# HengyiWang/spann3r

Hardware: NVIDIA H100
Metric: frames/sec (512x384, 10-frame seq) enc->mem-attn->dec->DPT (higher is better)
Workload: dtype bf16x3 (split-bf16 operands, fp32 accumulate; tf32 attention)

## Files before the change

### spann3r_b200/csrc/attention.cu

```cuda
#include "common.cuh"
#include "kernels.cuh"
#include "wgmma.cuh"

#include <cstdlib>
#include <cstring>

namespace s3r {

namespace attn {
constexpr int BQ = 128;
constexpr int BKV = 128;
constexpr int D = 64;
constexpr int Q_BYTES = BQ * D * 4;
constexpr int K_BYTES = BKV * D * 4;
constexpr int V_BYTES = D * BKV * 4;
constexpr int KV_STAGES = 3;
constexpr int SMEM = Q_BYTES + KV_STAGES * (K_BYTES + V_BYTES) + 1024 + 256;
constexpr int kThreads = 384;
constexpr int kConsumerWarps = 8;
}

__global__ void __launch_bounds__(attn::kThreads, 1) attention_kernel(const __grid_constant__ AttnArgs args) {
  using namespace attn;
  extern __shared__ uint8_t smem_raw[];
  uint8_t* smem = smem_raw + ((1024u - (smem_u32(smem_raw) & 1023u)) & 1023u);
  uint8_t* sQ = smem;
  uint8_t* sKV = sQ + Q_BYTES;
  uint64_t* bars = reinterpret_cast<uint64_t*>(sKV + KV_STAGES * (K_BYTES + V_BYTES));
  uint64_t* q_full = bars;
  uint64_t* kv_full = bars + 1;
  uint64_t* kv_empty = bars + 1 + KV_STAGES;

  const int warp = threadIdx.x >> 5, lane = threadIdx.x & 31;
  const int q0 = blockIdx.x * BQ;
  const int bh = blockIdx.y;
  const int nblk = (args.nk + BKV - 1) / BKV;

  if (warp == 0 && lane == 0) {
    tma_prefetch_desc(&args.tmQ);
    tma_prefetch_desc(&args.tmK);
    tma_prefetch_desc(&args.tmV);
    mbar_init(q_full, 1);
    for (int i = 0; i < KV_STAGES; ++i) {
      mbar_init(&kv_full[i], 1);
      mbar_init(&kv_empty[i], kConsumerWarps);
    }
    fence_barrier_init();
  }
  __syncthreads();
  pdl_launch_dependents();
  pdl_wait();

  if (warp < 4) {
    asm volatile("setmaxnreg.dec.sync.aligned.u32 40;");
    if (warp == 0 && lane == 0) {
      mbar_arrive_expect_tx(q_full, Q_BYTES);
      tma_load_3d(sQ, &args.tmQ, q_full, 0, q0, bh);
      tma_load_3d(sQ + Q_BYTES / 2, &args.tmQ, q_full, 32, q0, bh);
      for (int j = 0; j < nblk; ++j) {
        const int st = j % KV_STAGES;
        const uint32_t ph = (j / KV_STAGES) & 1;
        mbar_wait(&kv_empty[st], ph ^ 1);
        uint8_t* k = sKV + st * (K_BYTES + V_BYTES);
        uint8_t* v = k + K_BYTES;
        mbar_arrive_expect_tx(&kv_full[st], K_BYTES + V_BYTES);
        tma_load_3d(k, &args.tmK, &kv_full[st], 0, j * BKV, bh);
        tma_load_3d(k + K_BYTES / 2, &args.tmK, &kv_full[st], 32, j * BKV, bh);
#pragma unroll
        for (int a = 0; a < 4; ++a) tma_load_3d(v + a * (V_BYTES / 4), &args.tmV, &kv_full[st], j * BKV + a * 32, 0, bh);
      }
    }
    return;
  }

  asm volatile("setmaxnreg.inc.sync.aligned.u32 232;");
  const int wg = (warp - 4) >> 2;
  const int wq = warp & 3;
  const int g = lane >> 2, t4 = lane & 3;
  const uint32_t aQ = __shfl_sync(0xffffffffu, smem_u32(sQ), 0) + wg * (64 * 128);
  const uint32_t aKV = __shfl_sync(0xffffffffu, smem_u32(sKV), 0);
  constexpr float kLog2e = 1.4426950408889634f;

  float o[32];
#pragma unroll
  for (int i = 0; i < 32; ++i) o[i] = 0.f;
  float m0 = -INFINITY, m1 = -INFINITY, l0 = 0.f, l1 = 0.f;
  const int src_lo = (lane & ~3) | (t4 >> 1), src_hi = src_lo + 2;
  const bool odd = (t4 & 1) != 0;

  mbar_wait(q_full, 0);
  for (int j = 0; j < nblk; ++j) {
    const int st = j % KV_STAGES;
    mbar_wait(&kv_full[st], (j / KV_STAGES) & 1);
    const uint32_t aK = aKV + st * (K_BYTES + V_BYTES);
    const uint32_t aV = aK + K_BYTES;

    float s[64];
    wgmma_fence();
#pragma unroll
    for (int kk = 0; kk < 8; ++kk) {
      const uint32_t part = (kk >> 2) * (Q_BYTES / 2), ko = (kk & 3) * 2;
      wgmma_tf32_n128_ss(s, wgmma_desc_sw128_kmajor(aQ + part) + ko, wgmma_desc_sw128_kmajor(aK + part) + ko, kk > 0);
    }
    wgmma_commit();
    wgmma_wait<0>();

    const int kbase = j * BKV;
    if (kbase + BKV > args.nk) {
#pragma unroll
      for (int i = 0; i < 16; ++i) {
        const int c = kbase + 8 * i + 2 * t4;
        if (c >= args.nk) { s[4 * i] = -INFINITY; s[4 * i + 2] = -INFINITY; }
        if (c + 1 >= args.nk) { s[4 * i + 1] = -INFINITY; s[4 * i + 3] = -INFINITY; }
      }
    }
    float b0 = -INFINITY, b1 = -INFINITY;
#pragma unroll
    for (int i = 0; i < 16; ++i) {
      b0 = fmaxf(b0, fmaxf(s[4 * i], s[4 * i + 1]));
      b1 = fmaxf(b1, fmaxf(s[4 * i + 2], s[4 * i + 3]));
    }
#pragma unroll
    for (int x = 1; x < 4; x <<= 1) {
      b0 = fmaxf(b0, __shfl_xor_sync(0xffffffffu, b0, x));
      b1 = fmaxf(b1, __shfl_xor_sync(0xffffffffu, b1, x));
    }
    const float n0 = fmaxf(m0, b0), n1 = fmaxf(m1, b1);
    const float al0 = (j == 0) ? 0.f : exp2f((m0 - n0) * kLog2e);
    const float al1 = (j == 0) ? 0.f : exp2f((m1 - n1) * kLog2e);
    m0 = n0;
    m1 = n1;
    const float nr0 = -n0 * kLog2e, nr1 = -n1 * kLog2e;
    float ps0 = 0.f, ps1 = 0.f;
#pragma unroll
    for (int i = 0; i < 64; ++i) {
      const bool r1 = (i & 2) != 0;
      const float e = exp2f(fmaf(s[i], kLog2e, r1 ? nr1 : nr0));
      const uint32_t rb = (__float_as_uint(e) + 0x1000u) & 0xffffe000u;
      s[i] = __uint_as_float(rb);
      if (r1) ps1 += s[i]; else ps0 += s[i];
    }
    l0 = l0 * al0 + ps0;
    l1 = l1 * al1 + ps1;
#pragma unroll
    for (int i = 0; i < 8; ++i) {
      o[4 * i] *= al0; o[4 * i + 1] *= al0;
      o[4 * i + 2] *= al1; o[4 * i + 3] *= al1;
    }

    uint32_t pa[16][4];
#pragma unroll
    for (int kk = 0; kk < 16; ++kk) {
      const float x0 = __shfl_sync(0xffffffffu, s[4 * kk], src_lo), x1 = __shfl_sync(0xffffffffu, s[4 * kk + 1], src_lo);
      const float y0 = __shfl_sync(0xffffffffu, s[4 * kk + 2], src_lo), y1 = __shfl_sync(0xffffffffu, s[4 * kk + 3], src_lo);
      const float z0 = __shfl_sync(0xffffffffu, s[4 * kk], src_hi), z1 = __shfl_sync(0xffffffffu, s[4 * kk + 1], src_hi);
      const float w0 = __shfl_sync(0xffffffffu, s[4 * kk + 2], src_hi), w1 = __shfl_sync(0xffffffffu, s[4 * kk + 3], src_hi);
      pa[kk][0] = __float_as_uint(odd ? x1 : x0);
      pa[kk][1] = __float_as_uint(odd ? y1 : y0);
      pa[kk][2] = __float_as_uint(odd ? z1 : z0);
      pa[kk][3] = __float_as_uint(odd ? w1 : w0);
    }
    wgmma_fence();
#pragma unroll
    for (int kk = 0; kk < 16; ++kk)
      wgmma_tf32_n64_rs(o, pa[kk], wgmma_desc_sw128_kmajor(aV + (kk >> 2) * (V_BYTES / 4)) + (kk & 3) * 2, 1);
    wgmma_commit();
    wgmma_wait<0>();
    __syncwarp();
    if (lane == 0) mbar_arrive(&kv_empty[st]);
  }

#pragma unroll
  for (int x = 1; x < 4; x <<= 1) {
    l0 += __shfl_xor_sync(0xffffffffu, l0, x);
    l1 += __shfl_xor_sync(0xffffffffu, l1, x);
  }
  const float inv0 = 1.0f / l0, inv1 = 1.0f / l1;
  const int b = bh / args.heads, h = bh - b * args.heads;
#pragma unroll
  for (int r = 0; r < 2; ++r) {
    const int q = q0 + wg * 64 + wq * 16 + g + 8 * r;
    if (q >= args.nq) continue;
    const float inv = r ? inv1 : inv0;
    const long long row = ((long long)b * args.nq + q) * args.ldo + h * D;
#pragma unroll
    for (int i = 0; i < 8; ++i) {
      const float x = o[4 * i + 2 * r] * inv, y = o[4 * i + 2 * r + 1] * inv;
      const long long off = row + 8 * i + 2 * t4;
      if (args.o_f32) *reinterpret_cast<float2*>(args.o_f32 + off) = make_float2(x, y);
      if (args.o_hi) {
        uint32_t hh, ll;
        split2_bf16(x, y, hh, ll);
        *reinterpret_cast<uint32_t*>(args.o_hi + off) = hh;
        *reinterpret_cast<uint32_t*>(args.o_lo + off) = ll;
      }
    }
  }
}

int attn_plan_init(AttnPlan* plan, const float* q, const float* k, const float* vt, int BH, int heads, int nq, int nk,
                   int nk_pad) {
  using namespace attn;
  memset(plan, 0, sizeof(*plan));
  if (nk_pad % 4 != 0 || nk_pad < nk) {
    set_error("attention: nk_pad=%d must be >= nk=%d and a multiple of 4", nk_pad, nk);
    return -1;
  }
  AttnArgs& a = plan->args;
  {
    uint64_t dims[3] = {64, (uint64_t)nq, (uint64_t)BH};
    uint64_t str[2] = {64 * 4, (uint64_t)nq * 64 * 4};
    uint32_t box[3] = {32, (uint32_t)BQ, 1};
    int r = encode_tmap(&a.tmQ, CU_TENSOR_MAP_DATA_TYPE_FLOAT32, 3, q, dims, str, box);
    if (r) return r;
  }
  {
    uint64_t dims[3] = {64, (uint64_t)nk, (uint64_t)BH};
    uint64_t str[2] = {64 * 4, (uint64_t)nk * 64 * 4};
    uint32_t box[3] = {32, (uint32_t)BKV, 1};
    int r = encode_tmap(&a.tmK, CU_TENSOR_MAP_DATA_TYPE_FLOAT32, 3, k, dims, str, box);
    if (r) return r;
  }
  {
    uint64_t dims[3] = {(uint64_t)nk, 64, (uint64_t)BH};
    uint64_t str[2] = {(uint64_t)nk_pad * 4, (uint64_t)nk_pad * 64 * 4};
    uint32_t box[3] = {32, 64, 1};
    int r = encode_tmap(&a.tmV, CU_TENSOR_MAP_DATA_TYPE_FLOAT32, 3, vt, dims, str, box);
    if (r) return r;
  }
  a.nq = nq; a.nk = nk; a.heads = heads;
  plan->grid = dim3((nq + BQ - 1) / BQ, BH);
  plan->flops = 4.0 * BH * (double)nq * nk * 64;
  return 0;
}

static int attn_launch_args(const AttnPlan& plan, const AttnArgs& a, cudaStream_t st) {
  using namespace attn;
  static PerDeviceOnce once;
  bool& attr_set = once.cur();
  if (!attr_set) {
    cudaError_t e = cudaFuncSetAttribute(attention_kernel, cudaFuncAttributeMaxDynamicSharedMemorySize, SMEM);
    if (e != cudaSuccess) {
      set_error("attention: cudaFuncSetAttribute(smem=%d): %s", SMEM, cudaGetErrorString(e));
      return -5;
    }
    attr_set = true;
  }
  cudaError_t e = launch_pdl(attention_kernel, plan.grid, dim3(kThreads), SMEM, st, a);
  if (e != cudaSuccess) {
    set_error("attention launch failed: %s", cudaGetErrorString(e));
    return -6;
  }
  return 0;
}

int attn_launch(const AttnPlan& plan, __nv_bfloat16* o_hi, __nv_bfloat16* o_lo, float* o_f32, long long ldo,
                cudaStream_t st) {
  AttnArgs a = plan.args;
  a.o_hi = o_hi; a.o_lo = o_lo; a.o_f32 = o_f32; a.ldo = ldo;
  return attn_launch_args(plan, a, st);
}

int launch_attention(const float* q, const float* k, const float* vt, int BH, int heads, int nq, int nk, int nk_pad,
                     __nv_bfloat16* o_hi, __nv_bfloat16* o_lo, float* o_f32, long long ldo, cudaStream_t st) {
  if (heads <= 0 || BH % heads != 0 || ldo % 2 != 0) {
    set_error("attention: bh=%d must be a multiple of heads=%d, and ldo=%lld even (paired stores)", BH, heads, ldo);
    return -1;
  }
  if (nq <= 0 || nk <= 0 || BH <= 0) return 0;
  AttnPlan plan;
  int r = attn_plan_init(&plan, q, k, vt, BH, heads, nq, nk, nk_pad);
  if (r) return r;
  return attn_launch(plan, o_hi, o_lo, o_f32, ldo, st);
}

}
```

### spann3r_b200/csrc/common.cuh

```cuda
#pragma once
#include <cuda.h>
#include <cuda_bf16.h>
#include <cuda_runtime.h>
#include <stdint.h>

#include <cstdlib>
#include <utility>

namespace s3r {

__device__ __forceinline__ uint32_t smem_u32(const void* p) {
  return static_cast<uint32_t>(__cvta_generic_to_shared(p));
}
__device__ __forceinline__ uint32_t lane_id() { return threadIdx.x & 31; }
__device__ __forceinline__ bool elect_one() {
  uint32_t pred = 0;
  asm volatile(
      "{\n\t.reg .pred P1;\n\t"
      "elect.sync _|P1, 0xffffffff;\n\t"
      "selp.u32 %0, 1, 0, P1;\n\t}\n"
      : "=r"(pred));
  return pred != 0;
}

__device__ __forceinline__ void split_bf16(float x, __nv_bfloat16& hi, __nv_bfloat16& lo) {
  hi = __float2bfloat16_rn(x);
  lo = __float2bfloat16_rn(x - __bfloat162float(hi));
}
__device__ __forceinline__ void split2_bf16(float a, float b, uint32_t& hi, uint32_t& lo) {
  const __nv_bfloat162 h = __floats2bfloat162_rn(a, b);
  const uint32_t hu = *reinterpret_cast<const uint32_t*>(&h);
  const float ah = __uint_as_float(hu << 16), bh = __uint_as_float(hu & 0xffff0000u);
  const __nv_bfloat162 l = __floats2bfloat162_rn(a - ah, b - bh);
  hi = hu;
  lo = *reinterpret_cast<const uint32_t*>(&l);
}
__device__ __forceinline__ uint32_t pack_bf16(__nv_bfloat16 a, __nv_bfloat16 b) {
  return (uint32_t)__bfloat16_as_ushort(a) | ((uint32_t)__bfloat16_as_ushort(b) << 16);
}
__device__ __forceinline__ float to_tf32(float x) {
  uint32_t r;
  asm("cvt.rna.tf32.f32 %0, %1;" : "=r"(r) : "f"(x));
  return __uint_as_float(r);
}
__device__ __forceinline__ float gelu_erf1(float x) {
  return 0.5f * x * (1.0f + erff(x * 0.70710678118654752440f));
}
static __device__ __noinline__ float4 gelu_erf4(float4 x) {
  return make_float4(gelu_erf1(x.x), gelu_erf1(x.y), gelu_erf1(x.z), gelu_erf1(x.w));
}

__device__ __forceinline__ void mbar_init(uint64_t* bar, uint32_t count) {
  asm volatile("mbarrier.init.shared::cta.b64 [%0], %1;" ::"r"(smem_u32(bar)), "r"(count));
}
__device__ __forceinline__ void fence_barrier_init() {
  asm volatile("fence.mbarrier_init.release.cluster;" ::: "memory");
}
__device__ __forceinline__ void mbar_arrive_expect_tx(uint64_t* bar, uint32_t bytes) {
  asm volatile("mbarrier.arrive.expect_tx.shared::cta.b64 _, [%0], %1;" ::"r"(smem_u32(bar)), "r"(bytes)
               : "memory");
}
__device__ __forceinline__ void mbar_arrive(uint64_t* bar) {
  asm volatile("mbarrier.arrive.shared::cta.b64 _, [%0];" ::"r"(smem_u32(bar)) : "memory");
}
__device__ __forceinline__ bool mbar_try_wait(uint64_t* bar, uint32_t parity) {
  uint32_t ok;
  asm volatile(
      "{\n\t.reg .pred P1;\n\t"
      "mbarrier.try_wait.parity.shared::cta.b64 P1, [%1], %2;\n\t"
      "selp.u32 %0, 1, 0, P1;\n\t}\n"
      : "=r"(ok)
      : "r"(smem_u32(bar)), "r"(parity)
      : "memory");
  return ok != 0;
}
__device__ __forceinline__ void mbar_wait(uint64_t* bar, uint32_t parity) {
  uint32_t spins = 0;
  while (!mbar_try_wait(bar, parity)) {
    if (++spins > (1u << 28)) { asm volatile("trap;"); }
  }
}

__device__ __forceinline__ void fence_proxy_async_smem() {
  asm volatile("fence.proxy.async.shared::cta;" ::: "memory");
}
__device__ __forceinline__ void tma_prefetch_desc(const CUtensorMap* m) {
  asm volatile("prefetch.tensormap [%0];" ::"l"(reinterpret_cast<uint64_t>(m)) : "memory");
}
__device__ __forceinline__ void tma_load_2d(void* smem, const CUtensorMap* m, uint64_t* bar, int c0, int c1) {
  asm volatile(
      "cp.async.bulk.tensor.2d.shared::cta.global.mbarrier::complete_tx::bytes [%0], [%1, {%3, %4}], [%2];" ::"r"(
          smem_u32(smem)),
      "l"(reinterpret_cast<uint64_t>(m)), "r"(smem_u32(bar)), "r"(c0), "r"(c1)
      : "memory");
}
__device__ __forceinline__ void tma_load_3d(void* smem, const CUtensorMap* m, uint64_t* bar, int c0, int c1,
                                            int c2) {
  asm volatile(
      "cp.async.bulk.tensor.3d.shared::cta.global.mbarrier::complete_tx::bytes [%0], [%1, {%3, %4, %5}], [%2];" ::
          "r"(smem_u32(smem)),
      "l"(reinterpret_cast<uint64_t>(m)), "r"(smem_u32(bar)), "r"(c0), "r"(c1), "r"(c2)
      : "memory");
}
__device__ __forceinline__ void tma_load_4d(void* smem, const CUtensorMap* m, uint64_t* bar, int c0, int c1,
                                            int c2, int c3) {
  asm volatile(
      "cp.async.bulk.tensor.4d.shared::cta.global.mbarrier::complete_tx::bytes [%0], [%1, {%3, %4, %5, %6}], "
      "[%2];" ::"r"(smem_u32(smem)),
      "l"(reinterpret_cast<uint64_t>(m)), "r"(smem_u32(bar)), "r"(c0), "r"(c1), "r"(c2), "r"(c3)
      : "memory");
}

__device__ __forceinline__ void mbar_arrive_expect_tx_u(uint32_t bar, uint32_t bytes) {
  asm volatile("mbarrier.arrive.expect_tx.shared::cta.b64 _, [%0], %1;" ::"r"(bar), "r"(bytes) : "memory");
}
__device__ __forceinline__ void tma_load_3d_u(uint32_t smem, const CUtensorMap* m, uint32_t bar, int c0, int c1, int c2) {
  asm volatile(
      "cp.async.bulk.tensor.3d.shared::cta.global.mbarrier::complete_tx::bytes [%0], [%1, {%3, %4, %5}], [%2];" ::
          "r"(smem),
      "l"(reinterpret_cast<uint64_t>(m)), "r"(bar), "r"(c0), "r"(c1), "r"(c2)
      : "memory");
}
__device__ __forceinline__ void tma_load_4d_u(uint32_t smem, const CUtensorMap* m, uint32_t bar, int c0, int c1, int c2,
                                              int c3) {
  asm volatile(
      "cp.async.bulk.tensor.4d.shared::cta.global.mbarrier::complete_tx::bytes [%0], [%1, {%3, %4, %5, %6}], "
      "[%2];" ::"r"(smem),
      "l"(reinterpret_cast<uint64_t>(m)), "r"(bar), "r"(c0), "r"(c1), "r"(c2), "r"(c3)
      : "memory");
}

__device__ __forceinline__ uint64_t wgmma_desc_sw128_kmajor(uint32_t smem_addr) {
  uint64_t d = 0;
  d |= (uint64_t)((smem_addr & 0x3FFFF) >> 4);
  d |= (uint64_t)1 << 16;
  d |= (uint64_t)64 << 32;
  d |= (uint64_t)1 << 62;
  return d;
}

__device__ __forceinline__ uint64_t wgmma_desc_sw64_kmajor(uint32_t smem_addr) {
  uint64_t d = 0;
  d |= (uint64_t)((smem_addr & 0x3FFFF) >> 4);
  d |= (uint64_t)1 << 16;
  d |= (uint64_t)32 << 32;
  d |= (uint64_t)2 << 62;
  return d;
}

__device__ __forceinline__ void pdl_launch_dependents() { asm volatile("griddepcontrol.launch_dependents;" ::: "memory"); }
__device__ __forceinline__ void pdl_wait() { asm volatile("griddepcontrol.wait;" ::: "memory"); }

__device__ __forceinline__ unsigned long long globaltimer_ns() {
  unsigned long long t;
  asm volatile("mov.u64 %0, %%globaltimer;" : "=l"(t));
  return t;
}

__device__ __forceinline__ void st_f4(float* p, float a, float b, float c, float d) {
  *reinterpret_cast<float4*>(p) = make_float4(a, b, c, d);
}

struct PerDeviceOnce {
  bool done[64] = {};
  bool& cur() {
    int d = 0;
    cudaGetDevice(&d);
    return done[d & 63];
  }
};

template <typename... KArgs, typename... Args>
inline cudaError_t launch_pdl(void (*kernel)(KArgs...), dim3 grid, dim3 block, size_t smem, cudaStream_t st, Args&&... args) {
  cudaLaunchConfig_t cfg = {};
  cfg.gridDim = grid;
  cfg.blockDim = block;
  cfg.dynamicSmemBytes = smem;
  cfg.stream = st;
  static const bool use_pdl = (getenv("S3R_NO_PDL") == nullptr);
  cudaLaunchAttribute attr[1];
  attr[0].id = cudaLaunchAttributeProgrammaticStreamSerialization;
  attr[0].val.programmaticStreamSerializationAllowed = 1;
  cfg.attrs = attr;
  cfg.numAttrs = use_pdl ? 1 : 0;
  return cudaLaunchKernelEx(&cfg, kernel, std::forward<Args>(args)...);
}

}
```

### spann3r_b200/csrc/kernels.cuh

```cuda
#pragma once
#include <cuda_bf16.h>
#include <cuda_runtime.h>

#include "gemm.cuh"
#include <cuda.h>

struct s3r_loss_desc;
struct s3r_attn_train_desc;

namespace s3r {

int launch_split(const float* x, long long ldx, __nv_bfloat16* hi, __nv_bfloat16* lo, long long ldp, int col0,
                 long long rows, int C, int relu, cudaStream_t st);
int launch_split_stats(const float* x, long long ldx, long long rows, int C, float* out, long long ldo, __nv_bfloat16* hi,
                       __nv_bfloat16* lo, long long ldp, float2* stats, cudaStream_t st);
int launch_layernorm(const float* x, long long ldx, const float* w, const float* b, long long wb_group_stride,
                     long long rows_per_group, float eps, long long rows, int C, float* out, long long ldo,
                     __nv_bfloat16* hi, __nv_bfloat16* lo, long long ldp, int col0, long long swap_rows,
                     cudaStream_t st);
int launch_im2col_patch16(const float* img, long long sb, long long sc, long long sy, long long sx, int B, int gh,
                          int gw, __nv_bfloat16* hi, __nv_bfloat16* lo, cudaStream_t st);
int launch_im2col_3x3s2(const __nv_bfloat16* ihi, const __nv_bfloat16* ilo, int NB, int H, int W, int C, int Ho, int Wo,
                        __nv_bfloat16* ohi, __nv_bfloat16* olo, cudaStream_t st);
int launch_upsample2x(const float* x, int NB, int H, int W, int C, float* out, __nv_bfloat16* hi, __nv_bfloat16* lo,
                      cudaStream_t st, int Ho = 0, int Wo = 0);
int launch_rope2d(float* tokens, const long long* pos, long long BN, int H, int D, long long stride_tok,
                  long long stride_head, float base, float fwd, cudaStream_t st);

struct AttnArgs {
  alignas(64) CUtensorMap tmQ;
  alignas(64) CUtensorMap tmK;
  alignas(64) CUtensorMap tmV;
  int nq, nk, heads;
  __nv_bfloat16* o_hi;
  __nv_bfloat16* o_lo;
  float* o_f32;
  long long ldo;
};
struct AttnPlan {
  AttnArgs args;
  dim3 grid;
  double flops;
};
int attn_plan_init(AttnPlan* plan, const float* q, const float* k, const float* vt, int BH, int heads, int nq, int nk,
                   int nk_pad);
int attn_launch(const AttnPlan& plan, __nv_bfloat16* o_hi, __nv_bfloat16* o_lo, float* o_f32, long long ldo,
                cudaStream_t st);

constexpr int MEM_SOFTMAX_MAX_LEN = 200 * 1024 / 4;
constexpr int MEM_MAX_SLOTS = 64;
struct SlotInts {
  int n;
  int v[MEM_MAX_SLOTS];
  __host__ __device__ int operator[](int b) const { return v[n == 1 ? 0 : b]; }
};
inline SlotInts slot_uniform(int x) { SlotInts s{}; s.n = 1; s.v[0] = x; return s; }
int launch_mem_softmax(const float* S, long long ldS, long long rows, int nq, const SlotInts& lens, int Mmax, int Mpad,
                       float scale, float thresh, __nv_bfloat16* phi, __nv_bfloat16* plo, long long ldP, cudaStream_t st,
                       float drop_p = 0.f, unsigned long long seed = 0);
int launch_dropout_mask(float* out, long long n, unsigned long long seed, float p, cudaStream_t st);
int launch_mem_colsum(const __nv_bfloat16* phi, const __nv_bfloat16* plo, long long ldP, int B, int nq, const SlotInts& lens,
                      int Mmax, float* mem_attn, long long ld_attn, float* part, long long ld_part, cudaStream_t st);
int launch_split_transpose(const float* x, int B, int T, int C, __nv_bfloat16* ohi, __nv_bfloat16* olo, long long ldo,
                           long long out_batch_stride, const SlotInts& col0, const SlotInts& on, cudaStream_t st);
int launch_check_sim(const float* feat, const float* k, long long k_batch_stride, int B, const SlotInts& start,
                     const SlotInts& wm, int P, int C, float* scratch, float* out, int ldo, cudaStream_t st);

int launch_resample_h_u8(const uint8_t* src, long long row_stride, int rows, int out_cols, const int* bounds,
                         const int* kk, int ksize, int max_span, uint8_t* dst, cudaStream_t st);
int launch_resample_v_u8_norm(const uint8_t* tmp, int cols, int out_rows, const int* bounds, const int* kk, int ksize,
                              float* dst, cudaStream_t st);

int launch_focal_weiszfeld(const float* pts3d, int B, int H, int W, float ppx, float ppy, int iters, float lo, float hi,
                           float* scratch, float* focal, cudaStream_t st);

size_t pnp_workspace_bytes(int B, int n_samples);
int launch_pnp_ransac(const float* pts3d, const float* img_pts, int B, long long n, int width, double fx, double fy,
                      double cx, double cy, float reproj_err, int n_samples, int refine_iters, unsigned long long seed,
                      void* workspace, double* out, unsigned char* inlier_mask, cudaStream_t st);

int launch_focal_median(const float* pts3d, int B, int H, int W, float ppx, float ppy, float lo, float hi, int* scratch,
                        float* focal, cudaStream_t st);

int launch_conf_score(const float* conf, long long n, float* scratch256, float* out, cudaStream_t st);
int launch_conf_score_batched(const float* conf, int batch, long long hw, float* scratch, float* out, cudaStream_t st);

size_t pcl_index_bytes(long long n);
int launch_pcl_index_build(const void* pts, int f64, long long n, const double* T, void* index, cudaStream_t st);
int launch_pcl_nearest(const void* index, long long n, const void* q, int f64, long long nq, const double* T,
                       double max_dist, double* dist, long long* idx, cudaStream_t st);
int launch_pcl_normals(const void* index, long long n, int k, double* normals, cudaStream_t st);
size_t pcl_icp_workspace_bytes();
int launch_pcl_icp(const void* src, int f64, long long ns, const void* target_index, long long nt, double max_corr,
                   const double* init, int max_iteration, double rel_fitness, double rel_rmse, void* workspace,
                   double* out, cudaStream_t st);
size_t pcl_stats_workspace_bytes();
int launch_pcl_stats(const double* v, long long n, double threshold, void* workspace, double* out, cudaStream_t st);
int launch_pcl_abs_dot(const double* a, const double* b, const long long* idx, long long n, double* out, cudaStream_t st);

size_t render_workspace_bytes(int w, int h);
int launch_render_clear(void* keys, int w, int h, cudaStream_t st);
int launch_render_splat(const float* pts, const uint8_t* mask, long long n, long long id0, const double* camera,
                        double z_near, int w, int h, void* keys, cudaStream_t st);
int launch_render_resolve(const void* keys, const float* colors, int w, int h, uint8_t* out, cudaStream_t st);

size_t conv_wgrad_workspace_bytes(int NB, int H, int W, int N, int Kc, int taps);
int launch_conv_wgrad(const __nv_bfloat16* dy_hi, const __nv_bfloat16* dy_lo, long long ldy, const __nv_bfloat16* x_hi,
                      const __nv_bfloat16* x_lo, long long ldx, int NB, int H, int W, int N, int Kc, int taps,
                      void* workspace, size_t workspace_bytes, float* dw, cudaStream_t st);
int launch_col2im_3x3s2(const float* cols, int NB, int H, int W, int C, int Ho, int Wo, float* out, cudaStream_t st);

size_t loss_workspace_bytes(const s3r_loss_desc* d);
int launch_loss_forward(const s3r_loss_desc* d, void* ws, size_t ws_bytes, float* gt_out, float* pred_out,
                        uint8_t* valid_out, double* results, cudaStream_t st);
int launch_loss_backward(const s3r_loss_desc* d, const void* ws, size_t ws_bytes, const float* upstream,
                         float* grad_pred, float* grad_conf, cudaStream_t st);

int launch_attention(const float* q, const float* k, const float* vt, int BH, int heads, int nq, int nk, int nk_pad,
                     __nv_bfloat16* o_hi, __nv_bfloat16* o_lo, float* o_f32, long long ldo, cudaStream_t st);

size_t attn_train_workspace_bytes(const s3r_attn_train_desc* d);
int launch_attn_train_forward(const s3r_attn_train_desc* d, float* o, float* lse, cudaStream_t st);
int launch_attn_train_backward(const s3r_attn_train_desc* d, const float* o, const float* lse, const float* d_o,
                               void* workspace, size_t workspace_bytes, float* dq, float* dk, float* dv, cudaStream_t st);

}
```

Baseline: 92.83.

## Remove producer warpgroup, permute K rows via 5D TMA, overlap next QK^T with softmax

```diff
diff --git a/spann3r_b200/csrc/attention.cu b/spann3r_b200/csrc/attention.cu
--- a/spann3r_b200/csrc/attention.cu
+++ b/spann3r_b200/csrc/attention.cu
@@ -16,7 +16,7 @@
 constexpr int V_BYTES = D * BKV * 4;
 constexpr int KV_STAGES = 3;
 constexpr int SMEM = Q_BYTES + KV_STAGES * (K_BYTES + V_BYTES) + 1024 + 256;
-constexpr int kThreads = 384;
+constexpr int kThreads = 256;
 constexpr int kConsumerWarps = 8;
 }
 
@@ -39,6 +39,8 @@
   if (warp == 0 && lane == 0) {
     tma_prefetch_desc(&args.tmQ);
     tma_prefetch_desc(&args.tmK);
+    tma_prefetch_desc(&args.tmKlast);
+    tma_prefetch_desc(&args.tmKrow);
     tma_prefetch_desc(&args.tmV);
     mbar_init(q_full, 1);
     for (int i = 0; i < KV_STAGES; ++i) {
@@ -51,30 +53,7 @@
   pdl_launch_dependents();
   pdl_wait();
 
-  if (warp < 4) {
-    asm volatile("setmaxnreg.dec.sync.aligned.u32 40;");
-    if (warp == 0 && lane == 0) {
-      mbar_arrive_expect_tx(q_full, Q_BYTES);
-      tma_load_3d(sQ, &args.tmQ, q_full, 0, q0, bh);
-      tma_load_3d(sQ + Q_BYTES / 2, &args.tmQ, q_full, 32, q0, bh);
-      for (int j = 0; j < nblk; ++j) {
-        const int st = j % KV_STAGES;
-        const uint32_t ph = (j / KV_STAGES) & 1;
-        mbar_wait(&kv_empty[st], ph ^ 1);
-        uint8_t* k = sKV + st * (K_BYTES + V_BYTES);
-        uint8_t* v = k + K_BYTES;
-        mbar_arrive_expect_tx(&kv_full[st], K_BYTES + V_BYTES);
-        tma_load_3d(k, &args.tmK, &kv_full[st], 0, j * BKV, bh);
-        tma_load_3d(k + K_BYTES / 2, &args.tmK, &kv_full[st], 32, j * BKV, bh);
-#pragma unroll
-        for (int a = 0; a < 4; ++a) tma_load_3d(v + a * (V_BYTES / 4), &args.tmV, &kv_full[st], j * BKV + a * 32, 0, bh);
-      }
-    }
-    return;
-  }
-
-  asm volatile("setmaxnreg.inc.sync.aligned.u32 232;");
-  const int wg = (warp - 4) >> 2;
+  const int wg = warp >> 2;
   const int wq = warp & 3;
   const int g = lane >> 2, t4 = lane & 3;
   const uint32_t aQ = __shfl_sync(0xffffffffu, smem_u32(sQ), 0) + wg * (64 * 128);
@@ -85,17 +64,46 @@
 #pragma unroll
   for (int i = 0; i < 32; ++i) o[i] = 0.f;
   float m0 = -INFINITY, m1 = -INFINITY, l0 = 0.f, l1 = 0.f;
-  const int src_lo = (lane & ~3) | (t4 >> 1), src_hi = src_lo + 2;
-  const bool odd = (t4 & 1) != 0;
-
-  mbar_wait(q_full, 0);
-  for (int j = 0; j < nblk; ++j) {
+
+  const int ngrp = args.nk >> 3;
+  auto load_block = [&](int j) {
+    const int st = j % KV_STAGES;
+    mbar_wait(&kv_empty[st], ((j / KV_STAGES) & 1) ^ 1);
+    uint8_t* k = sKV + st * (K_BYTES + V_BYTES);
+    uint8_t* v = k + K_BYTES;
+    const int g0 = j * (BKV / 8);
+    if (g0 + BKV / 8 <= ngrp) {
+      mbar_arrive_expect_tx(&kv_full[st], K_BYTES + V_BYTES);
+      tma_load_5d(k, &args.tmK, &kv_full[st], 0, 0, 0, g0, bh);
+      tma_load_5d(k + K_BYTES / 2, &args.tmK, &kv_full[st], 32, 0, 0, g0, bh);
+    } else {
+      const int p = ngrp - g0, r = args.nk - 8 * ngrp;
+      mbar_arrive_expect_tx(&kv_full[st], (8 * p + r) * (2 * 128) + V_BYTES);
+      if (p > 0) {
+        tma_load_5d(k, &args.tmKlast, &kv_full[st], 0, 0, 0, g0, bh);
+        tma_load_5d(k + K_BYTES / 2, &args.tmKlast, &kv_full[st], 32, 0, 0, g0, bh);
+      }
+      for (int t = 0; t < r; ++t) {
+        const int row = 8 * p + 2 * (t & 3) + (t >> 2);
+        tma_load_3d(k + row * 128, &args.tmKrow, &kv_full[st], 0, 8 * ngrp + t, bh);
+        tma_load_3d(k + K_BYTES / 2 + row * 128, &args.tmKrow, &kv_full[st], 32, 8 * ngrp + t, bh);
+      }
+    }
+#pragma unroll
+    for (int a = 0; a < 4; ++a) tma_load_3d(v + a * (V_BYTES / 4), &args.tmV, &kv_full[st], j * BKV + a * 32, 0, bh);
+  };
+  if (threadIdx.x == 0) {
+    mbar_arrive_expect_tx(q_full, Q_BYTES);
+    tma_load_3d(sQ, &args.tmQ, q_full, 0, q0, bh);
+    tma_load_3d(sQ + Q_BYTES / 2, &args.tmQ, q_full, 32, q0, bh);
+    for (int j = 0; j < KV_STAGES && j < nblk; ++j) load_block(j);
+  }
+  __syncwarp();
+
+  auto issue_s = [&](float (&s)[64], int j) {
     const int st = j % KV_STAGES;
     mbar_wait(&kv_full[st], (j / KV_STAGES) & 1);
     const uint32_t aK = aKV + st * (K_BYTES + V_BYTES);
-    const uint32_t aV = aK + K_BYTES;
-
-    float s[64];
     wgmma_fence();
 #pragma unroll
     for (int kk = 0; kk < 8; ++kk) {
@@ -103,15 +111,21 @@
       wgmma_tf32_n128_ss(s, wgmma_desc_sw128_kmajor(aQ + part) + ko, wgmma_desc_sw128_kmajor(aK + part) + ko, kk > 0);
     }
     wgmma_commit();
-    wgmma_wait<0>();
+  };
+
+  auto kv_block = [&](float (&s)[64], float (&sn)[64], int j) {
+    if (threadIdx.x == 0 && j >= 1 && j + 2 < nblk) load_block(j + 2);
+    __syncwarp();
+    const int st = j % KV_STAGES;
+    const uint32_t aV = aKV + st * (K_BYTES + V_BYTES) + K_BYTES;
 
     const int kbase = j * BKV;
     if (kbase + BKV > args.nk) {
 #pragma unroll
       for (int i = 0; i < 16; ++i) {
-        const int c = kbase + 8 * i + 2 * t4;
+        const int c = kbase + 8 * i + t4;
         if (c >= args.nk) { s[4 * i] = -INFINITY; s[4 * i + 2] = -INFINITY; }
-        if (c + 1 >= args.nk) { s[4 * i + 1] = -INFINITY; s[4 * i + 3] = -INFINITY; }
+        if (c + 4 >= args.nk) { s[4 * i + 1] = -INFINITY; s[4 * i + 3] = -INFINITY; }
       }
     }
     float b0 = -INFINITY, b1 = -INFINITY;
@@ -130,6 +144,12 @@
     const float al1 = (j == 0) ? 0.f : exp2f((m1 - n1) * kLog2e);
     m0 = n0;
     m1 = n1;
+#pragma unroll
+    for (int i = 0; i < 8; ++i) {
+      o[4 * i] *= al0; o[4 * i + 1] *= al0;
+      o[4 * i + 2] *= al1; o[4 * i + 3] *= al1;
+    }
+    if (j + 1 < nblk) issue_s(sn, j + 1);
     const float nr0 = -n0 * kLog2e, nr1 = -n1 * kLog2e;
     float ps0 = 0.f, ps1 = 0.f;
 #pragma unroll
@@ -142,32 +162,28 @@
     }
     l0 = l0 * al0 + ps0;
     l1 = l1 * al1 + ps1;
-#pragma unroll
-    for (int i = 0; i < 8; ++i) {
-      o[4 * i] *= al0; o[4 * i + 1] *= al0;
-      o[4 * i + 2] *= al1; o[4 * i + 3] *= al1;
-    }
-
-    uint32_t pa[16][4];
+
+    wgmma_fence();
 #pragma unroll
     for (int kk = 0; kk < 16; ++kk) {
-      const float x0 = __shfl_sync(0xffffffffu, s[4 * kk], src_lo), x1 = __shfl_sync(0xffffffffu, s[4 * kk + 1], src_lo);
-      const float y0 = __shfl_sync(0xffffffffu, s[4 * kk + 2], src_lo), y1 = __shfl_sync(0xffffffffu, s[4 * kk + 3], src_lo);
-      const float z0 = __shfl_sync(0xffffffffu, s[4 * kk], src_hi), z1 = __shfl_sync(0xffffffffu, s[4 * kk + 1], src_hi);
-      const float w0 = __shfl_sync(0xffffffffu, s[4 * kk + 2], src_hi), w1 = __shfl_sync(0xffffffffu, s[4 * kk + 3], src_hi);
-      pa[kk][0] = __float_as_uint(odd ? x1 : x0);
-      pa[kk][1] = __float_as_uint(odd ? y1 : y0);
-      pa[kk][2] = __float_as_uint(odd ? z1 : z0);
-      pa[kk][3] = __float_as_uint(odd ? w1 : w0);
-    }
-    wgmma_fence();
-#pragma unroll
-    for (int kk = 0; kk < 16; ++kk)
-      wgmma_tf32_n64_rs(o, pa[kk], wgmma_desc_sw128_kmajor(aV + (kk >> 2) * (V_BYTES / 4)) + (kk & 3) * 2, 1);
+      const uint32_t pa[4] = {__float_as_uint(s[4 * kk]), __float_as_uint(s[4 * kk + 2]), __float_as_uint(s[4 * kk + 1]),
+                              __float_as_uint(s[4 * kk + 3])};
+      wgmma_tf32_n64_rs(o, pa, wgmma_desc_sw128_kmajor(aV + (kk >> 2) * (V_BYTES / 4)) + (kk & 3) * 2, 1);
+    }
     wgmma_commit();
     wgmma_wait<0>();
     __syncwarp();
     if (lane == 0) mbar_arrive(&kv_empty[st]);
+  };
+
+  float sa[64], sb[64];
+  mbar_wait(q_full, 0);
+  issue_s(sa, 0);
+  wgmma_wait<0>();
+  for (int j = 0; j < nblk; ++j) {
+    kv_block(sa, sb, j);
+#pragma unroll
+    for (int i = 0; i < 64; ++i) sa[i] = sb[i];
   }
 
 #pragma unroll
@@ -215,10 +231,20 @@
     if (r) return r;
   }
   {
-    uint64_t dims[3] = {64, (uint64_t)nk, (uint64_t)BH};
-    uint64_t str[2] = {64 * 4, (uint64_t)nk * 64 * 4};
-    uint32_t box[3] = {32, (uint32_t)BKV, 1};
-    int r = encode_tmap(&a.tmK, CU_TENSOR_MAP_DATA_TYPE_FLOAT32, 3, k, dims, str, box);
+    const int ngrp = nk / 8, nblk = (nk + BKV - 1) / BKV, plast = ngrp - (nblk - 1) * (BKV / 8);
+    const uint64_t row = 64 * 4;
+    uint64_t dims[5] = {64, 2, 4, (uint64_t)(ngrp > 0 ? ngrp : 1), (uint64_t)BH};
+    uint64_t str[4] = {4 * row, row, 8 * row, (uint64_t)nk * row};
+    uint32_t box[5] = {32, 2, 4, BKV / 8, 1};
+    int r = encode_tmap(&a.tmK, CU_TENSOR_MAP_DATA_TYPE_FLOAT32, 5, k, dims, str, box);
+    if (r) return r;
+    box[3] = (plast > 0 && plast < BKV / 8) ? (uint32_t)plast : BKV / 8;
+    r = encode_tmap(&a.tmKlast, CU_TENSOR_MAP_DATA_TYPE_FLOAT32, 5, k, dims, str, box);
+    if (r) return r;
+    uint64_t rdims[3] = {64, (uint64_t)nk, (uint64_t)BH};
+    uint64_t rstr[2] = {row, (uint64_t)nk * row};
+    uint32_t rbox[3] = {32, 1, 1};
+    r = encode_tmap(&a.tmKrow, CU_TENSOR_MAP_DATA_TYPE_FLOAT32, 3, k, rdims, rstr, rbox);
     if (r) return r;
   }
   {
diff --git a/spann3r_b200/csrc/common.cuh b/spann3r_b200/csrc/common.cuh
--- a/spann3r_b200/csrc/common.cuh
+++ b/spann3r_b200/csrc/common.cuh
@@ -110,6 +110,14 @@
       "l"(reinterpret_cast<uint64_t>(m)), "r"(smem_u32(bar)), "r"(c0), "r"(c1), "r"(c2), "r"(c3)
       : "memory");
 }
+__device__ __forceinline__ void tma_load_5d(void* smem, const CUtensorMap* m, uint64_t* bar, int c0, int c1,
+                                            int c2, int c3, int c4) {
+  asm volatile(
+      "cp.async.bulk.tensor.5d.shared::cta.global.mbarrier::complete_tx::bytes [%0], [%1, {%3, %4, %5, %6, %7}], "
+      "[%2];" ::"r"(smem_u32(smem)),
+      "l"(reinterpret_cast<uint64_t>(m)), "r"(smem_u32(bar)), "r"(c0), "r"(c1), "r"(c2), "r"(c3), "r"(c4)
+      : "memory");
+}
 
 __device__ __forceinline__ void mbar_arrive_expect_tx_u(uint32_t bar, uint32_t bytes) {
   asm volatile("mbarrier.arrive.expect_tx.shared::cta.b64 _, [%0], %1;" ::"r"(bar), "r"(bytes) : "memory");
diff --git a/spann3r_b200/csrc/kernels.cuh b/spann3r_b200/csrc/kernels.cuh
--- a/spann3r_b200/csrc/kernels.cuh
+++ b/spann3r_b200/csrc/kernels.cuh
@@ -30,6 +30,8 @@
 struct AttnArgs {
   alignas(64) CUtensorMap tmQ;
   alignas(64) CUtensorMap tmK;
+  alignas(64) CUtensorMap tmKlast;
+  alignas(64) CUtensorMap tmKrow;
   alignas(64) CUtensorMap tmV;
   int nq, nk, heads;
   __nv_bfloat16* o_hi;
```

Result: no change. 93.73 (median of 6 runs) (+1.0%).
